# zacz08/ADM

Hardware: AMD Instinct MI355X
Metric: train images/sec (CIFAR-10 32x32 uncond DDM UNet, 1 optimizer step/iter) + 10-step sample images/sec (higher is better)
Workload: dtype f32; 1 GPU; BASELINE configs[1]: CIFAR-10 32x32 uncond two-decoder DhariwalUNet (216M params), bs=128/GPU fp32, ddm_const schedule, dropout 0.1, loss_simple (LPIPS term needs unfetchable VGG16 weights), clip 1.0 + AdamW + EMA(every 8); global_batch=128, image=3x32x32, parallelism=dp1, valid=True

## Files before the change

### adm_amd/csrc/conv_gemm_x6.hip

```cpp
#include "common.h"
#include "../../include/adm_hip.h"

namespace {

struct G6P {
  const float* x; const unsigned short* w; const float* bias; const float* res; float* y;
  int M, N, K, ldx, ldy, ldr, wrows, tilesN, xbytes, wbytes, ybytes, rbytes;
  const float* amax_x; float wscale;
  float* amax_y;
};

typedef __attribute__((address_space(3))) void g6_lds_void;
typedef __bf16 bf16x8 __attribute__((ext_vector_type(8)));
typedef unsigned u32x2 __attribute__((ext_vector_type(2)));
typedef unsigned u32x4 __attribute__((ext_vector_type(4)));
typedef float f32x2 __attribute__((ext_vector_type(2)));
constexpr int GM = 128, GN = 128, GCH = 2;
template <int FMT> struct G6Fmt {
  static constexpr int TERMS = FMT ? 2 : 3;
  static constexpr int IMG = GCH * TERMS * 128 * 16;
  static constexpr int QW = 2 * TERMS;
};
typedef _Float16 g6_f16x8 __attribute__((ext_vector_type(8)));
typedef _Float16 g6_f16x2 __attribute__((ext_vector_type(2)));
__device__ inline float g6_scale(float amax) {
  if (!(amax > 0.f) || !(amax < 3e38f)) return 1.f;
  int e;
  frexpf(16000.f / amax, &e);
  return ldexpf(1.f, e - 1);
}
constexpr int G_RA = 2, G_RB = 4, G_D = 4;

__device__ __forceinline__ f32x4 g6_sub4(f32x4 a, f32x4 b) {
  f32x4 r;
#pragma unroll
  for (int i = 0; i < 4; ++i) asm("v_sub_f32 %0, %1, %2" : "=v"(r[i]) : "v"(a[i]), "v"(b[i]));
  return r;
}
__device__ __forceinline__ void g6_split3(const f32x4 v, u32x2& t0, u32x2& t1, u32x2& t2) {
  f32x4 h, mh;
#pragma unroll
  for (int i = 0; i < 4; ++i) h[i] = __uint_as_float(__float_as_uint(v[i]) & 0xFFFF0000u);
  const f32x4 r = g6_sub4(v, h);
#pragma unroll
  for (int i = 0; i < 4; ++i) mh[i] = __uint_as_float(__float_as_uint(r[i]) & 0xFFFF0000u);
  const f32x4 r2 = g6_sub4(r, mh);
  t0 = u32x2{__builtin_amdgcn_perm(__float_as_uint(v[1]), __float_as_uint(v[0]), 0x07060302u),
             __builtin_amdgcn_perm(__float_as_uint(v[3]), __float_as_uint(v[2]), 0x07060302u)};
  t1 = u32x2{__builtin_amdgcn_perm(__float_as_uint(r[1]), __float_as_uint(r[0]), 0x07060302u),
             __builtin_amdgcn_perm(__float_as_uint(r[3]), __float_as_uint(r[2]), 0x07060302u)};
  t2 = u32x2{__builtin_amdgcn_perm(__float_as_uint(r2[1]), __float_as_uint(r2[0]), 0x07060302u),
             __builtin_amdgcn_perm(__float_as_uint(r2[3]), __float_as_uint(r2[2]), 0x07060302u)};
}
__device__ __forceinline__ void g6_split2(const f32x4 v, float s, u32x2& t0, u32x2& t1) {
  _Float16 h0[4], h1[4];
#pragma unroll
  for (int i = 0; i < 4; ++i) {
    const float vs = v[i] * s;
    h0[i] = (_Float16)vs;
    h1[i] = (_Float16)(vs - (float)h0[i]);
  }
  t0 = u32x2{__builtin_bit_cast(unsigned, g6_f16x2{h0[0], h0[1]}), __builtin_bit_cast(unsigned, g6_f16x2{h0[2], h0[3]})};
  t1 = u32x2{__builtin_bit_cast(unsigned, g6_f16x2{h1[0], h1[1]}), __builtin_bit_cast(unsigned, g6_f16x2{h1[2], h1[3]})};
}
__device__ __forceinline__ void g6_barrier() {
  __builtin_amdgcn_fence(__ATOMIC_RELEASE, "workgroup", "local");
  __builtin_amdgcn_s_barrier();
  __builtin_amdgcn_fence(__ATOMIC_ACQUIRE, "workgroup", "local");
}

template <int FMT>
__global__ __launch_bounds__(512) void gemm_x6_kernel(G6P p) {
  constexpr int G_IMG = G6Fmt<FMT>::IMG, TERMS = G6Fmt<FMT>::TERMS, QW = G6Fmt<FMT>::QW;
  float sa = 1.f, inv_scale = 1.f;
  if (FMT) { sa = g6_scale(adm_amax_read(p.amax_x)); inv_scale = 1.f / (sa * p.wscale); }
  extern __shared__ __attribute__((aligned(16))) unsigned short smg[];
  unsigned short* As = smg;
  unsigned short* Bs = smg + G_RA * G_IMG;
  const int tid = threadIdx.x, lane = tid & 63, hw_wid = tid >> 6;
  const bool producer = hw_wid >= 4;
  const int wid = hw_wid & 3;
  int bid = blockIdx.x;
  {
    const int nwg = gridDim.x, q = nwg >> 3, r = nwg & 7, xcd = bid & 7, idx = bid >> 3;
    bid = (xcd < r ? xcd * (q + 1) : r * (q + 1) + (xcd - r) * q) + idx;
  }
  const int tilesM = gridDim.x / p.tilesN;
  const int tm = bid % tilesM, tn = bid / tilesM;
  const int m0 = tm * GM, n0 = tn * GN;
  const int S = p.K >> 5;
  constexpr unsigned OOB = 0x80000000u;

  if (producer) {
    const __amdgpu_buffer_rsrc_t rs_x = __builtin_amdgcn_make_buffer_rsrc(const_cast<float*>(p.x), 0, p.xbytes, 0x00020000);
    const int ptid = wid * 64 + lane;
    const int prow = ptid >> 3, quad = ptid & 7;
    unsigned voff[4];
#pragma unroll
    for (int j = 0; j < 4; ++j) {
      const int m = m0 + prow + 32 * j;
      voff[j] = (m < p.M) ? (unsigned)(((long)m * p.ldx + quad * 4) * 4) : OOB;
    }
    const int aq = quad & 3, ch = quad >> 2;
    unsigned short* la[4];
#pragma unroll
    for (int j = 0; j < 4; ++j) {
      const int row = prow + 32 * j;
      la[j] = As + (ch * TERMS * 128 + row) * 16 + ((((aq >> 1) ^ (row >> 3)) & 1) << 3) + (aq & 1) * 4;
    }
    f32x4 d[G_D][4];
    auto issue = [&](int set, int s) {
      const int soff = s << 7;
#pragma unroll
      for (int j = 0; j < 4; ++j)
        d[set][j] = __builtin_bit_cast(f32x4, __builtin_amdgcn_raw_buffer_load_b128(rs_x, (int)(s < S ? voff[j] : OOB), soff, 0));
    };
    auto store = [&](int set, int slot) {
#pragma unroll
      for (int j = 0; j < 4; ++j) {
        unsigned short* l = la[j] + slot * G_IMG;
        if (FMT) {
          u32x2 h0, h1;
          g6_split2(d[set][j], sa, h0, h1);
          *reinterpret_cast<u32x2*>(l) = h0;
          *reinterpret_cast<u32x2*>(l + 128 * 16) = h1;
          continue;
        }
        u32x2 t0, t1, t2;
        g6_split3(d[set][j], t0, t1, t2);
        *reinterpret_cast<u32x2*>(l) = t0;
        *reinterpret_cast<u32x2*>(l + 128 * 16) = t1;
        *reinterpret_cast<u32x2*>(l + 2 * 128 * 16) = t2;
      }
    };
#pragma unroll
    for (int k = 0; k < G_D; ++k) issue(k, k);
    __builtin_amdgcn_sched_barrier(0);
    for (int s0 = 0; s0 < S; s0 += G_D) {
#pragma unroll
      for (int k = 0; k < G_D; ++k) {
        if (s0 + k < S) {
          store(k, k & 1);
          __builtin_amdgcn_sched_barrier(0);
          issue(k, s0 + k + G_D);
          __builtin_amdgcn_sched_barrier(0);
          g6_barrier();
        }
      }
    }
    return;
  }

  const __amdgpu_buffer_rsrc_t rs_w = __builtin_amdgcn_make_buffer_rsrc(const_cast<unsigned short*>(p.w), 0, p.wbytes, 0x00020000);
  const int wm = wid >> 1, wn = wid & 1;
  const int lr = lane & 31, lh = lane >> 5;
  unsigned b_voff[QW];
#pragma unroll
  for (int i = 0; i < QW; ++i) {
    const int q = wid * QW + i, img = q >> 2;
    const int row = (q & 3) * 32 + (lane >> 1);
    const int n = n0 + row;
    const int half = (lane ^ (row >> 3)) & 1;
    b_voff[i] = (n < p.wrows) ? (unsigned)((((long)img * p.wrows + n) * 16 + half * 8) * 2) : OOB;
  }
  int ld_s = 0, ld_slot = 0;
  auto issue_b = [&]() {
    const int kb = (ld_s * GCH * TERMS * p.wrows) << 5;
    unsigned short* dst = Bs + ld_slot * G_IMG + (wid * QW) * 512;
#pragma unroll
    for (int i = 0; i < QW; ++i)
      __builtin_amdgcn_raw_ptr_buffer_load_lds(rs_w, (g6_lds_void*)(dst + i * 512), 16, (int)b_voff[i], kb, 0, 0);
    ++ld_s;
    if (++ld_slot == G_RB) ld_slot = 0;
  };

  f32x16 acc[2][2], tot[2][2];
#pragma unroll
  for (int a = 0; a < 2; ++a)
#pragma unroll
    for (int b = 0; b < 2; ++b)
#pragma unroll
      for (int r = 0; r < 16; ++r) tot[a][b][r] = 0.f;
  const int fh = ((lh ^ (lr >> 3)) & 1) * 8;
  const int a_foff = (wm * 64 + lr) * 16 + fh;
  const int b_foff = (wn * 64 + lr) * 16 + fh;
  const f32x16 zero = {0.f, 0.f, 0.f, 0.f, 0.f, 0.f, 0.f, 0.f, 0.f, 0.f, 0.f, 0.f, 0.f, 0.f, 0.f, 0.f};

  issue_b();
  if (S > 1) issue_b();
  if (S > 2) issue_b();
  int slot_b = 0;
  for (int s = 0; s < S; ++s) {
    if (s + 2 < S) { if (FMT) asm volatile("s_waitcnt vmcnt(8) lgkmcnt(0)\n\ts_barrier" ::: "memory"); else asm volatile("s_waitcnt vmcnt(12) lgkmcnt(0)\n\ts_barrier" ::: "memory"); }
    else if (s + 1 < S) { if (FMT) asm volatile("s_waitcnt vmcnt(4) lgkmcnt(0)\n\ts_barrier" ::: "memory"); else asm volatile("s_waitcnt vmcnt(6) lgkmcnt(0)\n\ts_barrier" ::: "memory"); }
    else asm volatile("s_waitcnt vmcnt(0) lgkmcnt(0)\n\ts_barrier" ::: "memory");
    if (s + 3 < S) issue_b();
    const unsigned short* Ab = As + (s & 1) * G_IMG + a_foff;
    const unsigned short* Bb = Bs + slot_b * G_IMG + b_foff;
    if (++slot_b == G_RB) slot_b = 0;
    const bool first = (s & 1) == 0;
#pragma unroll
    for (int ch = 0; ch < GCH; ++ch) {
      bf16x8 a[2][TERMS], b[2][TERMS];
#pragma unroll
      for (int k = 0; k < TERMS; ++k)
#pragma unroll
        for (int blk = 0; blk < 2; ++blk) {
          a[blk][k] = __builtin_bit_cast(bf16x8, *reinterpret_cast<const u32x4*>(Ab + ((ch * TERMS + k) * 128 + blk * 32) * 16));
          b[blk][k] = __builtin_bit_cast(bf16x8, *reinterpret_cast<const u32x4*>(Bb + ((ch * TERMS + k) * 128 + blk * 32) * 16));
        }
#pragma unroll
      for (int mi = 0; mi < 2; ++mi)
#pragma unroll
        for (int ni = 0; ni < 2; ++ni) {
          f32x16 c;
          if (FMT) {
            const g6_f16x8 a0 = __builtin_bit_cast(g6_f16x8, a[mi][0]), a1 = __builtin_bit_cast(g6_f16x8, a[mi][1]);
            const g6_f16x8 b0 = __builtin_bit_cast(g6_f16x8, b[ni][0]), b1 = __builtin_bit_cast(g6_f16x8, b[ni][1]);
            c = __builtin_amdgcn_mfma_f32_32x32x16_f16(a0, b1, (first && ch == 0) ? zero : acc[mi][ni], 0, 0, 0);
            c = __builtin_amdgcn_mfma_f32_32x32x16_f16(a1, b0, c, 0, 0, 0);
            acc[mi][ni] = __builtin_amdgcn_mfma_f32_32x32x16_f16(a0, b0, c, 0, 0, 0);
            continue;
          }
          if (first && ch == 0) c = __builtin_amdgcn_mfma_f32_32x32x16_bf16(a[mi][0], b[ni][TERMS - 1], zero, 0, 0, 0);
          else c = __builtin_amdgcn_mfma_f32_32x32x16_bf16(a[mi][0], b[ni][TERMS - 1], acc[mi][ni], 0, 0, 0);
#ifndef G6_HALF
          c = __builtin_amdgcn_mfma_f32_32x32x16_bf16(a[mi][TERMS - 1], b[ni][0], c, 0, 0, 0);
          c = __builtin_amdgcn_mfma_f32_32x32x16_bf16(a[mi][1], b[ni][1], c, 0, 0, 0);
          c = __builtin_amdgcn_mfma_f32_32x32x16_bf16(a[mi][0], b[ni][1], c, 0, 0, 0);
#endif
          c = __builtin_amdgcn_mfma_f32_32x32x16_bf16(a[mi][1], b[ni][0], c, 0, 0, 0);
          acc[mi][ni] = __builtin_amdgcn_mfma_f32_32x32x16_bf16(a[mi][0], b[ni][0], c, 0, 0, 0);
        }
    }
    if (!first || s + 1 == S) {
#pragma unroll
      for (int mi = 0; mi < 2; ++mi)
#pragma unroll
        for (int ni = 0; ni < 2; ++ni) tot[mi][ni] += acc[mi][ni];
    }
  }

  const __amdgpu_buffer_rsrc_t rs_y = __builtin_amdgcn_make_buffer_rsrc(p.y, 0, p.ybytes, 0x00020000);
  const __amdgpu_buffer_rsrc_t rs_r = __builtin_amdgcn_make_buffer_rsrc(const_cast<float*>(p.res), 0, p.res ? p.rbytes : 0, 0x00020000);
  float am = 0.f;
#pragma unroll
  for (int ni = 0; ni < 2; ++ni) {
    const int n = n0 + wn * 64 + ni * 32 + lr;
    const float bv = (p.bias && n < p.N) ? p.bias[n] : 0.f;
#pragma unroll
    for (int mi = 0; mi < 2; ++mi) {
      const int mb = m0 + wm * 64 + mi * 32 + 4 * lh;
      float rv[16];
      unsigned oy[16];
#pragma unroll
      for (int r = 0; r < 16; ++r) {
        const int m = mb + (r & 3) + 8 * (r >> 2);
        const bool ok = m < p.M && n < p.N;
        oy[r] = ok ? ((unsigned)m * (unsigned)p.ldy + (unsigned)n) * 4u : OOB;
        const unsigned orr = ok ? ((unsigned)m * (unsigned)p.ldr + (unsigned)n) * 4u : OOB;
        rv[r] = __builtin_bit_cast(float, __builtin_amdgcn_raw_buffer_load_b32(rs_r, (int)orr, 0, 0));
      }
#pragma unroll
      for (int r = 0; r < 16; ++r) {
        const float v = (FMT ? tot[mi][ni][r] * inv_scale : tot[mi][ni][r]) + bv + rv[r];
        if (oy[r] != OOB) am = fmaxf(am, fabsf(v));
        __builtin_amdgcn_raw_buffer_store_b32(__builtin_bit_cast(unsigned, v), rs_y, (int)oy[r], 0, 0);
      }
    }
  }
  adm_amax_commit(am, p.amax_y);
}

__global__ void split3_rows_kernel(const float* __restrict__ src, unsigned short* __restrict__ dst, int rows, int cols, int ld) {
  const long total = (long)rows * cols;
  for (long i = blockIdx.x * (long)blockDim.x + threadIdx.x; i < total; i += (long)gridDim.x * blockDim.x) {
    const int n = (int)(i / cols), c = (int)(i - (long)n * cols);
    const float a = src[(long)n * ld + c];
    const unsigned u = __float_as_uint(a);
    const float r = a - __uint_as_float(u & 0xFFFF0000u);
    const unsigned m = __float_as_uint(r);
    const float r2 = r - __uint_as_float(m & 0xFFFF0000u);
    unsigned short* d = dst + ((((long)(c >> 4) * 3) * rows + n) << 4) + (c & 15);
    const long term = (long)rows << 4;
    d[0] = (unsigned short)(u >> 16);
    d[term] = (unsigned short)(m >> 16);
    d[2 * term] = (unsigned short)(__float_as_uint(r2) >> 16);
  }
}

__global__ void split2_rows_kernel(const float* __restrict__ src, unsigned short* __restrict__ dst, int rows, int cols, int ld, float scale,
                                   int* __restrict__ overflow) {
  const long total = (long)rows * cols;
  bool bad = false;
  for (long i = blockIdx.x * (long)blockDim.x + threadIdx.x; i < total; i += (long)gridDim.x * blockDim.x) {
    const int n = (int)(i / cols), c = (int)(i - (long)n * cols);
    const float a = src[(long)n * ld + c] * scale;
    bad |= !(fabsf(a) < 65000.f);
    const _Float16 h0 = (_Float16)a, h1 = (_Float16)(a - (float)h0);
    unsigned short* d = dst + ((((long)(c >> 4) * 2) * rows + n) << 4) + (c & 15);
    d[0] = __builtin_bit_cast(unsigned short, h0);
    d[(long)rows << 4] = __builtin_bit_cast(unsigned short, h1);
  }
  if (bad && overflow) *overflow = 1;
}

}

extern "C" int adm_split3_rows(const float* src, void* dst, int rows, int cols, int ld, hipStream_t stream) {
  if (!src || !dst || rows <= 0 || cols <= 0 || (cols & 15) || ld < cols) return ADM_EINVAL;
  const long total = (long)rows * cols;
  const int grid = (int)((total + 255) / 256 > 4096 ? 4096 : (total + 255) / 256);
  hipLaunchKernelGGL(split3_rows_kernel, dim3(grid), dim3(256), 0, stream, src, static_cast<unsigned short*>(dst), rows, cols, ld);
  ADM_CHECK_LAUNCH();
  return ADM_OK;
}

static int gemm_x6_launch(const float* x, const void* w6, const float* bias, const float* res, float* y, long M, int K, int ldx, int N,
                          int wrows, int ldy, int ldr, hipStream_t stream, const float* amax_x, float wscale, float* amax_y) {
  const bool h3 = amax_x != nullptr;
  if (!x || !w6 || !y || M <= 0 || K <= 0 || (K & 31) || (ldx & 3) || N <= 0 || wrows < N) return ADM_EINVAL;
  if (((uintptr_t)x | (uintptr_t)w6) & 15) return ADM_EINVAL;
  if (h3 && !(wscale > 0.f)) return ADM_EINVAL;
  G6P p;
  p.x = x; p.w = static_cast<const unsigned short*>(w6); p.bias = bias; p.res = res; p.y = y;
  p.amax_x = amax_x; p.wscale = wscale; p.amax_y = amax_y;
  const long xb = M * ldx * 4, wb = (h3 ? 2L : 3L) * wrows * K * 2, yb = M * ldy * 4, rb = res ? M * ldr * 4 : 0;
  if (M >= (1L << 30) || xb >= (1L << 31) || wb >= (1L << 31) || yb >= (1L << 31) || rb >= (1L << 31)) return ADM_EINVAL;
  p.M = (int)M; p.N = N; p.K = K; p.ldx = ldx; p.ldy = ldy; p.ldr = ldr; p.wrows = wrows;
  p.xbytes = (int)xb; p.wbytes = (int)wb; p.ybytes = (int)yb; p.rbytes = (int)rb;
  p.tilesN = adm_cdiv(N, GN);
  constexpr int smem0 = (G_RA + G_RB) * G6Fmt<0>::IMG * (int)sizeof(unsigned short), smem1 = (G_RA + G_RB) * G6Fmt<1>::IMG * (int)sizeof(unsigned short);
  static bool attr_set = false;
  if (!attr_set) {
    if (hipFuncSetAttribute(reinterpret_cast<const void*>(&gemm_x6_kernel<0>), hipFuncAttributeMaxDynamicSharedMemorySize, smem0) != hipSuccess ||
        hipFuncSetAttribute(reinterpret_cast<const void*>(&gemm_x6_kernel<1>), hipFuncAttributeMaxDynamicSharedMemorySize, smem1) != hipSuccess)
      return ADM_ELAUNCH;
    attr_set = true;
  }
  const long grid = (long)adm_cdiv(M, GM) * p.tilesN;
  if (h3) hipLaunchKernelGGL(gemm_x6_kernel<1>, dim3((unsigned)grid), dim3(512), smem1, stream, p);
  else hipLaunchKernelGGL(gemm_x6_kernel<0>, dim3((unsigned)grid), dim3(512), smem0, stream, p);
  ADM_CHECK_LAUNCH();
  return ADM_OK;
}

extern "C" int adm_gemm_x6(const float* x, const void* w6, const float* bias, const float* res, float* y, long M, int K, int ldx, int N,
                           int wrows, int ldy, int ldr, hipStream_t stream) {
  return gemm_x6_launch(x, w6, bias, res, y, M, K, ldx, N, wrows, ldy, ldr, stream, nullptr, 0.f, nullptr);
}
extern "C" int adm_gemm_x6_amax(const float* x, const void* w6, const float* bias, const float* res, float* y, long M, int K, int ldx, int N,
                                int wrows, int ldy, int ldr, float* amax_y, hipStream_t stream) {
  return gemm_x6_launch(x, w6, bias, res, y, M, K, ldx, N, wrows, ldy, ldr, stream, nullptr, 0.f, amax_y);
}
extern "C" int adm_gemm_x6_h3(const float* x, const void* wh, const float* bias, const float* res, float* y, long M, int K, int ldx, int N,
                              int wrows, int ldy, int ldr, const float* amax_x, float wscale, float* amax_y, hipStream_t stream) {
  if (!amax_x) return ADM_EINVAL;
  return gemm_x6_launch(x, wh, bias, res, y, M, K, ldx, N, wrows, ldy, ldr, stream, amax_x, wscale, amax_y);
}
extern "C" int adm_split2_rows_f16(const float* src, void* dst, int rows, int cols, int ld, float scale, int* overflow, hipStream_t stream) {
  if (!src || !dst || rows <= 0 || cols <= 0 || (cols & 15) || ld < cols || !(scale > 0.f)) return ADM_EINVAL;
  const long total = (long)rows * cols;
  const int grid = (int)((total + 255) / 256 > 4096 ? 4096 : (total + 255) / 256);
  hipLaunchKernelGGL(split2_rows_kernel, dim3(grid), dim3(256), 0, stream, src, static_cast<unsigned short*>(dst), rows, cols, ld, scale, overflow);
  ADM_CHECK_LAUNCH();
  return ADM_OK;
}
```

### adm_amd/hip.py

```python
from __future__ import annotations

import ctypes
import os
import subprocess
from ctypes import c_double, c_float, c_int, c_long, c_uint64, c_void_p

import torch

_HERE = os.path.dirname(os.path.abspath(__file__))
LIB_PATH = os.path.join(_HERE, "libadm_hip.so")
_lib = None

P, I, L, F, D, U = c_void_p, c_int, c_long, c_float, c_double, c_uint64
_SIGS = {
    "adm_version": [],
    "adm_conv_fwd": [P, P, P, P, P, I, I, I, I, I, I, I, I, I, I, I, I, P],
    "adm_conv_splitk": [I, I, I],
    "adm_conv_fwd_ws": [P, P, P, P, P, P, L, I, I, I, I, I, I, I, I, I, I, I, P],
    "adm_conv_fwd_strided": [P, P, P, P, P, I, I, I, I, I, I, I, I, I, I, I, I, I, I, P],
    "adm_conv_fwd_wino": [P, P, P, P, P, I, I, I, I, I, I, I, I, I, P],
    "adm_conv_fwd_wino_up": [P, P, P, P, P, I, I, I, I, I, I, I, I, I, P],
    "adm_pack_weight_wino": [P, P, P, I, I, I, I, P],
    "adm_pack_weight_wino2d": [P, P, P, I, I, I, I, P],
    "adm_conv_fwd_wino2d": [P, P, P, P, P, P, L, I, I, I, I, I, I, I, I, I, P],
    "adm_wino2d_splitk": [I, I, I, I, I],
    "adm_wino2d_variant": [I],
    "adm_wino2d_h3_wide": [I],
    "adm_wgrad_h3_blocks": [I],
    "adm_conv_fwd_wino2d_x6": [P, P, P, P, P, P, L, I, I, I, I, I, I, I, I, I, P],
    "adm_conv_fwd_wino2d_x6_up": [P, P, P, P, P, P, L, I, I, I, I, I, I, I, I, I, P],
    "adm_wino2d_x6_splitk": [I, I, I, I, I],
    "adm_split3_bf16": [P, P, I, I, P],
    "adm_split2_f16": [P, P, I, I, F, P, P],
    "adm_conv_fwd_wino2d_h3": [P, P, P, P, P, P, L, I, I, I, I, I, I, I, I, I, P, F, I, P],
    "adm_gemm_x6": [P, P, P, P, P, L, I, I, I, I, I, I, P],
    "adm_gemm_x6_amax": [P, P, P, P, P, L, I, I, I, I, I, I, P, P],
    "adm_gemm_x6_h3": [P, P, P, P, P, L, I, I, I, I, I, I, P, F, P, P],
    "adm_split2_rows_f16": [P, P, I, I, I, F, P, P],
    "adm_split3_rows": [P, P, I, I, I, P],
    "adm_conv_wgrad_x6": [P, P, P, P, I, I, I, I, I, I, I, I, P],
    "adm_conv_wgrad_x6_up": [P, P, P, P, I, I, I, I, I, I, I, I, P],
    "adm_conv_wgrad_x6_ws": [P, P, P, P, I, I, I, I, I, I, I, I, I, P],
    "adm_conv_wgrad_x6_plan": [I, I, I, I, I],
    "adm_gemm_wgrad_x6": [P, P, P, P, L, I, I, I, I, I, P],
    "adm_gemm_wgrad_x6_ws": [P, P, P, P, L, I, I, I, I, I, P],
    "adm_gemm_wgrad_x6_plan": [L, I, I],
    "adm_conv_wgrad_x6_h3": [P, P, P, P, I, I, I, I, I, I, I, I, I, I, P, P, P],
    "adm_gemm_wgrad_x6_h3": [P, P, P, P, L, I, I, I, I, I, I, P, P, P],
    "adm_conv_wgrad_x6_bf16a": [P, P, P, P, I, I, I, I, I, I, I, I, I, P],
    "adm_gemm_wgrad_x6_bf16a": [P, P, P, P, L, I, I, I, I, I, P],
    "adm_conv_wgrad": [P, P, P, I, I, I, I, I, I, I, I, I, I, P],
    "adm_conv_wgrad_wino": [P, P, P, P, I, I, I, I, I, I, I, I, P],
    "adm_conv_wgrad_wino_up": [P, P, P, P, I, I, I, I, I, I, I, I, P],
    "adm_conv_wgrad_bias": [P, P, P, P, I, I, I, I, I, I, I, I, I, I, P],
    "adm_conv_wgrad_wino2d": [P, P, P, P, I, I, I, I, I, I, I, I, P],
    "adm_unpack_wgrad_wino2d": [P, I, P, I, I, I, I, I, P, P, P],
    "adm_conv_wgrad_plan": [I, I, I, I, I, I, I, I],
    "adm_conv_wgrad_ws": [P, P, P, P, I, I, I, I, I, I, I, I, I, I, I, P],
    "adm_unpack_wgrad_splits": [P, I, P, I, I, I, I, I, I, I, P, P, P],
    "adm_conv_fwd_bf16": [P, P, P, P, P, I, I, I, I, I, I, I, I, I, I, I, I, P],
    "adm_conv_wgrad_bf16": [P, P, P, I, I, I, I, I, I, I, I, I, I, P],
    "adm_conv_fwd_bf16a": [P, P, P, P, P, I, I, I, I, I, I, I, I, I, I, I, I, P],
    "adm_conv_wgrad_bf16a": [P, P, P, I, I, I, I, I, I, I, I, I, I, P],
    "adm_gn_fwd_bf16out": [P, P, P, P, P, P, L, P, I, I, I, I, F, I, F, U, P],
    "adm_f32_to_bf16": [P, P, L, P],
    "adm_pack_weight": [P, P, P, I, I, I, I, I, I, P],
    "adm_pack_weight_table": [P, I, L, P],
    "adm_unpack_wgrad_table": [P, I, L, P],
    "adm_gn_bwd_param_table": [P, I, L, P],
    "adm_unpack_wgrad": [P, P, I, I, I, I, I, I, I, P],
    "adm_permute_vec": [P, P, I, I, I, I, P],
    "adm_colsum": [P, P, I, I, I, I, P],
    "adm_gn_splits": [I, I],
    "adm_gn_fused": [I],
    "adm_gn_stats": [P, P, P, I, I, I, I, F, P],
    "adm_gn_apply": [P, P, P, P, P, L, P, I, I, I, I, I, F, U, P],
    "adm_gn_fwd": [P, P, P, P, P, P, L, P, I, I, I, I, F, I, F, U, P],
    "adm_gn_fwd_amax": [P, P, P, P, P, P, L, P, P, I, I, I, I, F, I, F, U, P],
    "adm_gn_bwd": [P, P, P, P, P, P, L, P, P, P, P, P, I, I, I, I, I, F, U, P],
    "adm_gn_bwd_add": [P, P, P, P, P, P, L, P, P, P, P, P, P, I, I, I, I, I, F, U, P],
    "adm_gn_bwd_add_amax": [P, P, P, P, P, P, L, P, P, P, P, P, P, P, I, I, I, I, I, F, U, P],
    "adm_softmax_rows": [P, L, I, L, F, P],
    "adm_posterior_sample": [P, I, P, P, I, L, I, F, P],
    "adm_attn_fwd": [P, P, P, I, I, I, P],
    "adm_attn_bwd": [P, P, P, P, P, P, I, I, I, P],
    "adm_attn_bwd_amax": [P, P, P, P, P, P, P, I, I, I, P],
    "adm_attn_fwd_h3": [P, P, P, P, I, I, I, P],
    "adm_attn_bwd_h3": [P, P, P, P, P, P, P, P, P, I, I, I, P],
    "adm_resample2x": [P, P, I, I, I, I, I, F, I, P],
    "adm_nchw_to_nhwc": [P, I, P, L, P, I, I, I, I, P],
    "adm_nchw_to_nhwc_amax": [P, I, P, L, P, P, I, I, I, I, P],
# ... 70 lines not shown
    "adm_transpose2d": [P, P, I, I, P],
    "adm_adaptive_weight": [P, L, P, L, P, F, P, P],
    "adm_axpy_dev": [P, P, P, F, P, L, P],
    "adm_swin_attn_fwd": [P, P, P, P, I, I, I, I, I, I, I, I, P],
    "adm_ln_affine_fwd": [P, P, P, P, L, I, F, P],
    "adm_swin_merge_ln_fwd": [P, P, P, P, I, I, I, I, F, P],
    "adm_swin_attn_bwd_ws_floats": [I, I, I, I],
    "adm_swin_attn_bwd": [P, P, P, P, P, P, P, P, I, I, I, I, I, I, I, I, I, I, P],
    "adm_ln_bwd_ws_floats": [L, I],
    "adm_ln_affine_bwd": [P, P, P, P, P, P, P, L, I, F, I, P],
    "adm_swin_merge_ln_bwd": [P, P, P, P, P, P, P, I, I, I, I, F, I, P],
    "adm_rowscale_add": [P, P, P, P, I, L, P],
}
EXPORTS = tuple(_SIGS)


def build(verbose: bool = False) -> str:
    r = subprocess.run(["make", "-C", os.path.join(_HERE, "csrc"), "-j8"], capture_output=True, text=True)
    if verbose or r.returncode != 0:
        print(r.stdout[-4000:], r.stderr[-8000:])
    if r.returncode != 0 or not os.path.exists(LIB_PATH):
        raise RuntimeError("building libadm_hip.so failed")
    return LIB_PATH


def lib() -> ctypes.CDLL:
    global _lib
    if _lib is None:
        if not os.path.exists(LIB_PATH):
            raise RuntimeError(f"{LIB_PATH} is missing: run `python -c 'import __graft_entry__ as g; g.build()'` "
                               "(there is no non-HIP fallback for the adm_amd hot path)")
        _lib = ctypes.CDLL(LIB_PATH)
        for name, args in _SIGS.items():
            fn = getattr(_lib, name)
            fn.argtypes = args
            fn.restype = c_long if name in ("adm_aug_workspace_floats", "adm_linattn_ws_floats", "adm_swin_attn_bwd_ws_floats",
                                        "adm_ln_bwd_ws_floats") else c_int
        if os.environ.get("ADM_H3_WIDE") is not None:
            _lib.adm_wino2d_h3_wide(int(os.environ["ADM_H3_WIDE"]))
        if os.environ.get("ADM_WGRAD_H3_BLOCKS") is not None:
            _lib.adm_wgrad_h3_blocks(int(os.environ["ADM_WGRAD_H3_BLOCKS"]))
    return _lib


def stream() -> c_void_p:
    return c_void_p(torch.cuda.current_stream().cuda_stream)


def ptr(t) -> c_void_p:
    return None if t is None else c_void_p(t.data_ptr())


NO_STREAM = ("adm_version", "adm_conv_splitk", "adm_gn_splits", "adm_aug_workspace_floats", "adm_conv_wgrad_plan",
             "adm_sumsq_blocks", "adm_lnc_blocks", "adm_bn_blocks", "adm_linattn_ws_floats", "adm_wino2d_splitk", "adm_wino2d_x6_splitk", "adm_wino2d_variant", "adm_wino2d_h3_wide", "adm_wgrad_h3_blocks", "adm_gn_fused", "adm_conv_wgrad_x6_plan", "adm_gemm_wgrad_x6_plan", "adm_lpips_head_blocks", "adm_ae_blocks", "adm_swin_attn_bwd_ws_floats", "adm_ln_bwd_ws_floats")


def call(name: str, *args):
    rc = getattr(lib(), name)(*args, stream())
    if rc != 0:
        raise RuntimeError(f"{name} failed with code {rc} (-22 = unsupported shape/alignment, -5 = launch failure)")


def require_cuda(t: torch.Tensor, what: str = "tensor"):
    if not t.is_cuda:
        raise RuntimeError(f"adm_amd: {what} is on {t.device}; the HIP hot path needs a GPU tensor "
                           "(no CPU fallback exists by design)")
```

### include/adm_hip.h

```cpp
#ifndef ADM_HIP_H
#define ADM_HIP_H
#include <stdint.h>
typedef struct ihipStream_t* hipStream_t;

#ifdef __cplusplus
#define ADM_AMAX_SLOTS 64
#define ADM_AMAX_STRIDE 32
#define ADM_AMAX_FLOATS (ADM_AMAX_SLOTS * ADM_AMAX_STRIDE)

extern "C" {
#endif

int adm_version(void);


int adm_conv_fwd(const float* x, const float* wp, const float* bias, const float* res, float* y,
                 int B, int H, int W, int Cin, int ldx, int N, int wrows, int ldy, int ldr,
                 int ks, int up, int tile, hipStream_t stream);

int adm_conv_fwd_strided(const float* x, const float* wp, const float* bias, const float* res, float* y,
                         int B, int Hin, int Win, int Hout, int Wout, int Cin, int ldx, int N, int wrows,
                         int ldy, int ldr, int ks, int stride, int pad_lo, hipStream_t stream);

int adm_conv_fwd_wino(const float* x, const float* wq, const float* bias, const float* res, float* y, int B, int H, int W,
                      int Cin, int ldx, int N, int wrows, int ldy, int ldr, hipStream_t stream);
int adm_conv_fwd_wino_up(const float* x, const float* wq, const float* bias, const float* res, float* y, int B, int H, int W,
                         int Cin, int ldx, int N, int wrows, int ldy, int ldr, hipStream_t stream);
int adm_pack_weight_wino(const float* w, float* wf, float* wb, int Co, int Ci, int Co_pad, int Ci_pad, hipStream_t stream);

int adm_conv_splitk(int M, int N, int K);
int adm_conv_fwd_ws(const float* x, const float* wp, const float* bias, const float* res, float* y, float* ws,
                    long ws_floats, int B, int H, int W, int Cin, int ldx, int N, int wrows, int ldy, int ldr, int ks,
                    int up, hipStream_t stream);

int adm_conv_wgrad(const float* x, const float* dy, float* dwp, int B, int H, int W, int Cin, int ldx,
                   int Cout, int lddy, int ks, int up, int splits, hipStream_t stream);

int adm_conv_wgrad_bias(const float* x, const float* dy, float* dwp, float* dbias, int B, int H, int W, int Cin, int ldx,
                        int Cout, int lddy, int ks, int up, int splits, hipStream_t stream);

int adm_conv_wgrad_wino(const float* x, const float* dy, float* dwp, float* dbias, int B, int H, int W, int Cin, int ldx,
                        int Cout, int lddy, int splits, hipStream_t stream);

int adm_conv_wgrad_wino_up(const float* x, const float* dy, float* dwp, float* dbias, int B, int H, int W, int Cin, int ldx,
                           int Cout, int lddy, int splits, hipStream_t stream);

int adm_pack_weight_wino2d(const float* w, float* wf, float* wb, int Co, int Ci, int Co_pad, int Ci_pad, hipStream_t stream);
int adm_conv_fwd_wino2d(const float* x, const float* wq, const float* bias, const float* res, float* y, float* ws, long ws_floats,
                        int B, int H, int W, int Cin, int ldx, int N, int wrows, int ldy, int ldr, hipStream_t stream);
int adm_conv_fwd_wino2d_x6(const float* x, const void* wq6, const float* bias, const float* res, float* y, float* ws,
                           long ws_floats, int B, int H, int W, int Cin, int ldx, int N, int wrows, int ldy, int ldr,
                           hipStream_t stream);
int adm_conv_fwd_wino2d_x6_up(const float* x, const void* wq6, const float* bias, const float* res, float* y, float* ws,
                              long ws_floats, int B, int H, int W, int Cin, int ldx, int N, int wrows, int ldy, int ldr,
                              hipStream_t stream);
int adm_wino2d_x6_splitk(int B, int H, int W, int Cin, int N);
int adm_split2_f16(const float* src, void* dst, int rows, int cols, float scale, int* overflow, hipStream_t stream);
int adm_conv_fwd_wino2d_h3(const float* x, const void* wqh, const float* bias, const float* res, float* y, float* ws,
                           long ws_floats, int B, int H, int W, int Cin, int ldx, int N, int wrows, int ldy, int ldr,
                           const float* amax_x, float wscale, int up, hipStream_t stream);
int adm_split3_bf16(const float* src, void* dst, int rows, int cols, hipStream_t stream);
int adm_gemm_x6(const float* x, const void* w6, const float* bias, const float* res, float* y, long M, int K, int ldx, int N, int wrows,
                int ldy, int ldr, hipStream_t stream);
int adm_split3_rows(const float* src, void* dst, int rows, int cols, int ld, hipStream_t stream);
int adm_gemm_x6_amax(const float* x, const void* w6, const float* bias, const float* res, float* y, long M, int K, int ldx, int N,
                     int wrows, int ldy, int ldr, float* amax_y, hipStream_t stream);
int adm_gemm_x6_h3(const float* x, const void* wh, const float* bias, const float* res, float* y, long M, int K, int ldx, int N, int wrows,
                   int ldy, int ldr, const float* amax_x, float wscale, float* amax_y, hipStream_t stream);
int adm_split2_rows_f16(const float* src, void* dst, int rows, int cols, int ld, float scale, int* overflow, hipStream_t stream);
int adm_conv_wgrad_x6(const float* x, const float* dy, float* dwp2, float* dbias, int B, int H, int W, int Cin, int ldx, int Cout,
                      int lddy, int splits, hipStream_t stream);
int adm_conv_wgrad_x6_up(const float* x, const float* dy, float* dwp2, float* dbias, int B, int H, int W, int Cin, int ldx, int Cout,
                         int lddy, int splits, hipStream_t stream);
int adm_conv_wgrad_x6_ws(const float* x, const float* dy, float* ws, float* bws, int B, int H, int W, int Cin, int ldx, int Cout,
                         int lddy, int splits, int up, hipStream_t stream);
int adm_conv_wgrad_x6_plan(int B, int H, int W, int Cin, int Cout);
int adm_gemm_wgrad_x6(const float* x, const float* dy, float* dwp, float* dbias, long P, int Cin, int ldx, int Cout, int lddy,
                      int splits, hipStream_t stream);
int adm_gemm_wgrad_x6_ws(const float* x, const float* dy, float* ws, float* bws, long P, int Cin, int ldx, int Cout, int lddy,
                         int splits, hipStream_t stream);
int adm_gemm_wgrad_x6_plan(long P, int Cin, int Cout);
int adm_conv_wgrad_x6_bf16a(const void* x16, const float* dy, float* dwp2, float* dbias, int B, int H, int W, int Cin, int ldx,
                            int Cout, int lddy, int splits, int up, hipStream_t stream);
int adm_gemm_wgrad_x6_bf16a(const void* x16, const float* dy, float* dwp, float* dbias, long P, int Cin, int ldx, int Cout, int lddy,
                            int splits, hipStream_t stream);
int adm_conv_wgrad_x6_h3(const float* x, const float* dy, float* dwp2, float* dbias, int B, int H, int W, int Cin, int ldx, int Cout,
                         int lddy, int splits, int up, int det, const float* amax_x, const float* amax_dy, hipStream_t stream);
int adm_gemm_wgrad_x6_h3(const float* x, const float* dy, float* dwp, float* dbias, long P, int Cin, int ldx, int Cout, int lddy,
                         int splits, int det, const float* amax_x, const float* amax_dy, hipStream_t stream);
int adm_wino2d_variant(int ws);
int adm_wino2d_h3_wide(int v);
int adm_wgrad_h3_blocks(int v);
int adm_wino2d_splitk(int B, int H, int W, int Cin, int N);

int adm_conv_wgrad_wino2d(const float* x, const float* dy, float* dwp2, float* dbias, int B, int H, int W, int Cin, int ldx,
                          int Cout, int lddy, int splits, hipStream_t stream);
int adm_unpack_wgrad_wino2d(const float* wx, int splits, float* dw, int Co, int Ci, int Co_pad, int Ci_pad, int accumulate,
                            const float* bws, float* dbias, hipStream_t stream);

int adm_conv_wgrad_plan(int B, int H, int W, int Cin, int Cout, int ks, int up, int wino);
int adm_conv_wgrad_ws(const float* x, const float* dy, float* ws, float* bws, int B, int H, int W, int Cin, int ldx, int Cout,
                      int lddy, int ks, int up, int splits, int wino, hipStream_t stream);

int adm_conv_fwd_bf16(const float* x, const unsigned short* wp16, const float* bias, const float* res, float* y,
                      int B, int H, int W, int Cin, int ldx, int N, int wrows, int ldy, int ldr, int ks, int up,
                      int tile, hipStream_t stream);
int adm_conv_wgrad_bf16(const float* x, const float* dy, float* dwp, int B, int H, int W, int Cin, int ldx, int Cout,
                        int lddy, int ks, int up, int splits, hipStream_t stream);
int adm_conv_fwd_bf16a(const void* x16, const unsigned short* wp16, const float* bias, const float* res, float* y, int B, int H, int W,
                       int Cin, int ldx, int N, int wrows, int ldy, int ldr, int ks, int up, int tile, hipStream_t stream);
int adm_conv_wgrad_bf16a(const void* x16, const float* dy, float* dwp, int B, int H, int W, int Cin, int ldx, int Cout, int lddy, int ks,
                         int up, int splits, hipStream_t stream);
int adm_gn_fwd_bf16out(const float* x, float* stats, double* ws, const float* gamma, const float* beta, const float* ss,
                       long ss_bstride, void* y16, int B, int HW, int C, int G, float eps, int silu, float drop_p, uint64_t seed,
                       hipStream_t stream);
int adm_f32_to_bf16(const float* src, unsigned short* dst, long n, hipStream_t stream);

int adm_pack_weight(const float* w, float* wp_fwd, float* wp_bwd, int Co, int Ci, int ks, int Co_pad, int Ci_pad,
                    int qkv, hipStream_t stream);
int adm_pack_weight_table(const long* table, int n_entries, long total_tiles, hipStream_t stream);
int adm_unpack_wgrad(const float* dwp, float* dw, int Co, int Ci, int ks, int Co_pad, int Ci_pad, int qkv,
                     int accumulate, hipStream_t stream);
// ... 232 lines not shown
```

Baseline: 1249 images/s.

## Make x6 GEMM kernel process multiple output tiles per workgroup to fix wave quantization

The split-bf16 GEMM kernel now lets each workgroup loop over a chunk of T consecutive output tiles instead of exactly one. A host-side planner picks T so the number of rounds over 256 concurrent workgroups is no worse than launching one tile per workgroup. The producer and consumer pipelines carry their K-step and tile counters across tile boundaries, with a full drain barrier at each new tile and the epilogue run per tile. This targets tail-wave imbalance on large tile counts, at the cost of extra index bookkeeping, a pipeline stall at each tile switch, and some ablation macros left in the code.

```diff
diff --git a/adm_amd/csrc/conv_gemm_x6.hip b/adm_amd/csrc/conv_gemm_x6.hip
--- a/adm_amd/csrc/conv_gemm_x6.hip
+++ b/adm_amd/csrc/conv_gemm_x6.hip
@@ -5,7 +5,7 @@
 
 struct G6P {
   const float* x; const unsigned short* w; const float* bias; const float* res; float* y;
-  int M, N, K, ldx, ldy, ldr, wrows, tilesN, xbytes, wbytes, ybytes, rbytes;
+  int M, N, K, ldx, ldy, ldr, wrows, tilesM, tilesN, tiles, T, xbytes, wbytes, ybytes, rbytes;
   const float* amax_x; float wscale;
   float* amax_y;
 };
@@ -30,6 +30,9 @@
   return ldexpf(1.f, e - 1);
 }
 constexpr int G_RA = 2, G_RB = 4, G_D = 4;
+#ifndef G6_ABL
+#define G6_ABL 0
+#endif
 
 __device__ __forceinline__ f32x4 g6_sub4(f32x4 a, f32x4 b) {
   f32x4 r;
@@ -80,27 +83,32 @@
   const int tid = threadIdx.x, lane = tid & 63, hw_wid = tid >> 6;
   const bool producer = hw_wid >= 4;
   const int wid = hw_wid & 3;
-  int bid = blockIdx.x;
+  int c = blockIdx.x;
   {
-    const int nwg = gridDim.x, q = nwg >> 3, r = nwg & 7, xcd = bid & 7, idx = bid >> 3;
-    bid = (xcd < r ? xcd * (q + 1) : r * (q + 1) + (xcd - r) * q) + idx;
-  }
-  const int tilesM = gridDim.x / p.tilesN;
-  const int tm = bid % tilesM, tn = bid / tilesM;
-  const int m0 = tm * GM, n0 = tn * GN;
-  const int S = p.K >> 5;
+    const int nwg = gridDim.x, q = nwg >> 3, r = nwg & 7, xcd = c & 7, idx = c >> 3;
+    c = (xcd < r ? xcd * (q + 1) : r * (q + 1) + (xcd - r) * q) + idx;
+  }
+  const int t0 = c * p.T;
+  const int nT = min(p.T, p.tiles - t0);
+  const int S = (G6_ABL & 1) ? 0 : p.K >> 5;
+  const int G = nT * S;
   constexpr unsigned OOB = 0x80000000u;
 
   if (producer) {
+    if (G6_ABL & 1) return;
     const __amdgpu_buffer_rsrc_t rs_x = __builtin_amdgcn_make_buffer_rsrc(const_cast<float*>(p.x), 0, p.xbytes, 0x00020000);
     const int ptid = wid * 64 + lane;
     const int prow = ptid >> 3, quad = ptid & 7;
+    int is_ = 0, ij = 0, im = t0 % p.tilesM;
     unsigned voff[4];
-#pragma unroll
-    for (int j = 0; j < 4; ++j) {
-      const int m = m0 + prow + 32 * j;
-      voff[j] = (m < p.M) ? (unsigned)(((long)m * p.ldx + quad * 4) * 4) : OOB;
-    }
+    auto tile_rows = [&]() {
+#pragma unroll
+      for (int j = 0; j < 4; ++j) {
+        const int m = im * GM + prow + 32 * j;
+        voff[j] = (ij < nT && m < p.M) ? ((unsigned)m * (unsigned)p.ldx + quad * 4) * 4u : OOB;
+      }
+    };
+    tile_rows();
     const int aq = quad & 3, ch = quad >> 2;
     unsigned short* la[4];
 #pragma unroll
@@ -109,11 +117,16 @@
       la[j] = As + (ch * TERMS * 128 + row) * 16 + ((((aq >> 1) ^ (row >> 3)) & 1) << 3) + (aq & 1) * 4;
     }
     f32x4 d[G_D][4];
-    auto issue = [&](int set, int s) {
-      const int soff = s << 7;
+    auto issue = [&](int set) {
+      const int soff = is_ << 7;
 #pragma unroll
       for (int j = 0; j < 4; ++j)
-        d[set][j] = __builtin_bit_cast(f32x4, __builtin_amdgcn_raw_buffer_load_b128(rs_x, (int)(s < S ? voff[j] : OOB), soff, 0));
+        d[set][j] = __builtin_bit_cast(f32x4, __builtin_amdgcn_raw_buffer_load_b128(rs_x, (int)voff[j], soff, 0));
+      if (++is_ == S) {
+        is_ = 0; ++ij;
+        if (++im == p.tilesM) im = 0;
+        tile_rows();
+      }
     };
     auto store = [&](int set, int slot) {
 #pragma unroll
@@ -126,23 +139,23 @@
           *reinterpret_cast<u32x2*>(l + 128 * 16) = h1;
           continue;
         }
-        u32x2 t0, t1, t2;
-        g6_split3(d[set][j], t0, t1, t2);
-        *reinterpret_cast<u32x2*>(l) = t0;
+        u32x2 t0_, t1, t2;
+        g6_split3(d[set][j], t0_, t1, t2);
+        *reinterpret_cast<u32x2*>(l) = t0_;
         *reinterpret_cast<u32x2*>(l + 128 * 16) = t1;
         *reinterpret_cast<u32x2*>(l + 2 * 128 * 16) = t2;
       }
     };
 #pragma unroll
-    for (int k = 0; k < G_D; ++k) issue(k, k);
+    for (int k = 0; k < G_D; ++k) issue(k);
     __builtin_amdgcn_sched_barrier(0);
-    for (int s0 = 0; s0 < S; s0 += G_D) {
+    for (int g0 = 0; g0 < G; g0 += G_D) {
 #pragma unroll
       for (int k = 0; k < G_D; ++k) {
-        if (s0 + k < S) {
+        if (g0 + k < G) {
           store(k, k & 1);
           __builtin_amdgcn_sched_barrier(0);
-          issue(k, s0 + k + G_D);
+          issue(k);
           __builtin_amdgcn_sched_barrier(0);
           g6_barrier();
         }
@@ -154,24 +167,31 @@
   const __amdgpu_buffer_rsrc_t rs_w = __builtin_amdgcn_make_buffer_rsrc(const_cast<unsigned short*>(p.w), 0, p.wbytes, 0x00020000);
   const int wm = wid >> 1, wn = wid & 1;
   const int lr = lane & 31, lh = lane >> 5;
+  int tm = t0 % p.tilesM, tn = t0 / p.tilesM;
+  int ld_s = 0, ld_slot = 0, ld_tm = tm, ld_tn = tn;
   unsigned b_voff[QW];
-#pragma unroll
-  for (int i = 0; i < QW; ++i) {
-    const int q = wid * QW + i, img = q >> 2;
-    const int row = (q & 3) * 32 + (lane >> 1);
-    const int n = n0 + row;
-    const int half = (lane ^ (row >> 3)) & 1;
-    b_voff[i] = (n < p.wrows) ? (unsigned)((((long)img * p.wrows + n) * 16 + half * 8) * 2) : OOB;
-  }
-  int ld_s = 0, ld_slot = 0;
+  auto tile_cols = [&]() {
+#pragma unroll
+    for (int i = 0; i < QW; ++i) {
+      const int q = wid * QW + i, img = q >> 2;
+      const int row = (q & 3) * 32 + (lane >> 1);
+      const int n = ld_tn * GN + row;
+      const int half = (lane ^ (row >> 3)) & 1;
+      b_voff[i] = (n < p.wrows) ? (unsigned)((((long)img * p.wrows + n) * 16 + half * 8) * 2) : OOB;
+    }
+  };
+  tile_cols();
   auto issue_b = [&]() {
     const int kb = (ld_s * GCH * TERMS * p.wrows) << 5;
     unsigned short* dst = Bs + ld_slot * G_IMG + (wid * QW) * 512;
 #pragma unroll
     for (int i = 0; i < QW; ++i)
       __builtin_amdgcn_raw_ptr_buffer_load_lds(rs_w, (g6_lds_void*)(dst + i * 512), 16, (int)b_voff[i], kb, 0, 0);
-    ++ld_s;
     if (++ld_slot == G_RB) ld_slot = 0;
+    if (++ld_s == S) {
+      ld_s = 0;
+      if (++ld_tm == p.tilesM) { ld_tm = 0; ++ld_tn; tile_cols(); }
+    }
   };
 
   f32x16 acc[2][2], tot[2][2];
@@ -185,89 +205,106 @@
   const int a_foff = (wm * 64 + lr) * 16 + fh;
   const int b_foff = (wn * 64 + lr) * 16 + fh;
   const f32x16 zero = {0.f, 0.f, 0.f, 0.f, 0.f, 0.f, 0.f, 0.f, 0.f, 0.f, 0.f, 0.f, 0.f, 0.f, 0.f, 0.f};
-
-  issue_b();
-  if (S > 1) issue_b();
-  if (S > 2) issue_b();
-  int slot_b = 0;
-  for (int s = 0; s < S; ++s) {
-    if (s + 2 < S) { if (FMT) asm volatile("s_waitcnt vmcnt(8) lgkmcnt(0)\n\ts_barrier" ::: "memory"); else asm volatile("s_waitcnt vmcnt(12) lgkmcnt(0)\n\ts_barrier" ::: "memory"); }
-    else if (s + 1 < S) { if (FMT) asm volatile("s_waitcnt vmcnt(4) lgkmcnt(0)\n\ts_barrier" ::: "memory"); else asm volatile("s_waitcnt vmcnt(6) lgkmcnt(0)\n\ts_barrier" ::: "memory"); }
-    else asm volatile("s_waitcnt vmcnt(0) lgkmcnt(0)\n\ts_barrier" ::: "memory");
-    if (s + 3 < S) issue_b();
-    const unsigned short* Ab = As + (s & 1) * G_IMG + a_foff;
-    const unsigned short* Bb = Bs + slot_b * G_IMG + b_foff;
-    if (++slot_b == G_RB) slot_b = 0;
-    const bool first = (s & 1) == 0;
-#pragma unroll
-    for (int ch = 0; ch < GCH; ++ch) {
-      bf16x8 a[2][TERMS], b[2][TERMS];
-#pragma unroll
-      for (int k = 0; k < TERMS; ++k)
-#pragma unroll
-        for (int blk = 0; blk < 2; ++blk) {
-          a[blk][k] = __builtin_bit_cast(bf16x8, *reinterpret_cast<const u32x4*>(Ab + ((ch * TERMS + k) * 128 + blk * 32) * 16));
-          b[blk][k] = __builtin_bit_cast(bf16x8, *reinterpret_cast<const u32x4*>(Bb + ((ch * TERMS + k) * 128 + blk * 32) * 16));
-        }
-#pragma unroll
-      for (int mi = 0; mi < 2; ++mi)
-#pragma unroll
-        for (int ni = 0; ni < 2; ++ni) {
-          f32x16 c;
-          if (FMT) {
-            const g6_f16x8 a0 = __builtin_bit_cast(g6_f16x8, a[mi][0]), a1 = __builtin_bit_cast(g6_f16x8, a[mi][1]);
-            const g6_f16x8 b0 = __builtin_bit_cast(g6_f16x8, b[ni][0]), b1 = __builtin_bit_cast(g6_f16x8, b[ni][1]);
-            c = __builtin_amdgcn_mfma_f32_32x32x16_f16(a0, b1, (first && ch == 0) ? zero : acc[mi][ni], 0, 0, 0);
-            c = __builtin_amdgcn_mfma_f32_32x32x16_f16(a1, b0, c, 0, 0, 0);
-            acc[mi][ni] = __builtin_amdgcn_mfma_f32_32x32x16_f16(a0, b0, c, 0, 0, 0);
-            continue;
-          }
-          if (first && ch == 0) c = __builtin_amdgcn_mfma_f32_32x32x16_bf16(a[mi][0], b[ni][TERMS - 1], zero, 0, 0, 0);
-          else c = __builtin_amdgcn_mfma_f32_32x32x16_bf16(a[mi][0], b[ni][TERMS - 1], acc[mi][ni], 0, 0, 0);
-#ifndef G6_HALF
-          c = __builtin_amdgcn_mfma_f32_32x32x16_bf16(a[mi][TERMS - 1], b[ni][0], c, 0, 0, 0);
-          c = __builtin_amdgcn_mfma_f32_32x32x16_bf16(a[mi][1], b[ni][1], c, 0, 0, 0);
-          c = __builtin_amdgcn_mfma_f32_32x32x16_bf16(a[mi][0], b[ni][1], c, 0, 0, 0);
-#endif
-          c = __builtin_amdgcn_mfma_f32_32x32x16_bf16(a[mi][1], b[ni][0], c, 0, 0, 0);
-          acc[mi][ni] = __builtin_amdgcn_mfma_f32_32x32x16_bf16(a[mi][0], b[ni][0], c, 0, 0, 0);
-        }
-    }
-    if (!first || s + 1 == S) {
-#pragma unroll
-      for (int mi = 0; mi < 2; ++mi)
-#pragma unroll
-        for (int ni = 0; ni < 2; ++ni) tot[mi][ni] += acc[mi][ni];
-    }
-  }
-
   const __amdgpu_buffer_rsrc_t rs_y = __builtin_amdgcn_make_buffer_rsrc(p.y, 0, p.ybytes, 0x00020000);
   const __amdgpu_buffer_rsrc_t rs_r = __builtin_amdgcn_make_buffer_rsrc(const_cast<float*>(p.res), 0, p.res ? p.rbytes : 0, 0x00020000);
   float am = 0.f;
-#pragma unroll
-  for (int ni = 0; ni < 2; ++ni) {
-    const int n = n0 + wn * 64 + ni * 32 + lr;
-    const float bv = (p.bias && n < p.N) ? p.bias[n] : 0.f;
-#pragma unroll
-    for (int mi = 0; mi < 2; ++mi) {
-      const int mb = m0 + wm * 64 + mi * 32 + 4 * lh;
-      float rv[16];
-      unsigned oy[16];
-#pragma unroll
-      for (int r = 0; r < 16; ++r) {
-        const int m = mb + (r & 3) + 8 * (r >> 2);
-        const bool ok = m < p.M && n < p.N;
-        oy[r] = ok ? ((unsigned)m * (unsigned)p.ldy + (unsigned)n) * 4u : OOB;
-        const unsigned orr = ok ? ((unsigned)m * (unsigned)p.ldr + (unsigned)n) * 4u : OOB;
-        rv[r] = __builtin_bit_cast(float, __builtin_amdgcn_raw_buffer_load_b32(rs_r, (int)orr, 0, 0));
-      }
-#pragma unroll
-      for (int r = 0; r < 16; ++r) {
-        const float v = (FMT ? tot[mi][ni][r] * inv_scale : tot[mi][ni][r]) + bv + rv[r];
-        if (oy[r] != OOB) am = fmaxf(am, fabsf(v));
-        __builtin_amdgcn_raw_buffer_store_b32(__builtin_bit_cast(unsigned, v), rs_y, (int)oy[r], 0, 0);
-      }
-    }
+
+  if (G > 0) issue_b();
+  if (G > 1) issue_b();
+  if (G > 2) issue_b();
+  int g = 0, slot_b = 0;
+  for (int j = 0; j < nT; ++j) {
+    for (int s = 0; s < S; ++s, ++g) {
+      if (s == 0 && j > 0) asm volatile("s_waitcnt vmcnt(0) lgkmcnt(0)\n\ts_barrier" ::: "memory");
+      else if (g + 2 < G) { if (FMT) asm volatile("s_waitcnt vmcnt(8) lgkmcnt(0)\n\ts_barrier" ::: "memory"); else asm volatile("s_waitcnt vmcnt(12) lgkmcnt(0)\n\ts_barrier" ::: "memory"); }
+      else if (g + 1 < G) { if (FMT) asm volatile("s_waitcnt vmcnt(4) lgkmcnt(0)\n\ts_barrier" ::: "memory"); else asm volatile("s_waitcnt vmcnt(6) lgkmcnt(0)\n\ts_barrier" ::: "memory"); }
+      else asm volatile("s_waitcnt vmcnt(0) lgkmcnt(0)\n\ts_barrier" ::: "memory");
+      if (g + 3 < G) issue_b();
+      const unsigned short* Ab = As + (g & 1) * G_IMG + a_foff;
+      const unsigned short* Bb = Bs + slot_b * G_IMG + b_foff;
+      if (++slot_b == G_RB) slot_b = 0;
+      const bool first = (s & 1) == 0;
+#pragma unroll
+      for (int ch = 0; ch < GCH; ++ch) {
+        bf16x8 a[2][TERMS], b[2][TERMS];
+#pragma unroll
+        for (int k = 0; k < TERMS; ++k)
+#pragma unroll
+          for (int blk = 0; blk < 2; ++blk) {
+            a[blk][k] = __builtin_bit_cast(bf16x8, *reinterpret_cast<const u32x4*>(Ab + ((ch * TERMS + k) * 128 + blk * 32) * 16));
+            b[blk][k] = __builtin_bit_cast(bf16x8, *reinterpret_cast<const u32x4*>(Bb + ((ch * TERMS + k) * 128 + blk * 32) * 16));
+          }
+#pragma unroll
+        for (int mi = 0; mi < 2; ++mi)
+#pragma unroll
+          for (int ni = 0; ni < 2; ++ni) {
+            f32x16 c_;
+            if (FMT) {
+              const g6_f16x8 a0 = __builtin_bit_cast(g6_f16x8, a[mi][0]), a1 = __builtin_bit_cast(g6_f16x8, a[mi][1]);
+              const g6_f16x8 b0 = __builtin_bit_cast(g6_f16x8, b[ni][0]), b1 = __builtin_bit_cast(g6_f16x8, b[ni][1]);
+              c_ = __builtin_amdgcn_mfma_f32_32x32x16_f16(a0, b1, (first && ch == 0) ? zero : acc[mi][ni], 0, 0, 0);
+              c_ = __builtin_amdgcn_mfma_f32_32x32x16_f16(a1, b0, c_, 0, 0, 0);
+              acc[mi][ni] = __builtin_amdgcn_mfma_f32_32x32x16_f16(a0, b0, c_, 0, 0, 0);
+              continue;
+            }
+            if (first && ch == 0) c_ = __builtin_amdgcn_mfma_f32_32x32x16_bf16(a[mi][0], b[ni][TERMS - 1], zero, 0, 0, 0);
+            else c_ = __builtin_amdgcn_mfma_f32_32x32x16_bf16(a[mi][0], b[ni][TERMS - 1], acc[mi][ni], 0, 0, 0);
+#ifndef G6_HALF
+            c_ = __builtin_amdgcn_mfma_f32_32x32x16_bf16(a[mi][TERMS - 1], b[ni][0], c_, 0, 0, 0);
+            c_ = __builtin_amdgcn_mfma_f32_32x32x16_bf16(a[mi][1], b[ni][1], c_, 0, 0, 0);
+            c_ = __builtin_amdgcn_mfma_f32_32x32x16_bf16(a[mi][0], b[ni][1], c_, 0, 0, 0);
+#endif
+            c_ = __builtin_amdgcn_mfma_f32_32x32x16_bf16(a[mi][1], b[ni][0], c_, 0, 0, 0);
+            acc[mi][ni] = __builtin_amdgcn_mfma_f32_32x32x16_bf16(a[mi][0], b[ni][0], c_, 0, 0, 0);
+          }
+      }
+      if (!first || s + 1 == S) {
+#pragma unroll
+        for (int mi = 0; mi < 2; ++mi)
+#pragma unroll
+          for (int ni = 0; ni < 2; ++ni) tot[mi][ni] += acc[mi][ni];
+      }
+    }
+
+    const int m0 = tm * GM, n0 = tn * GN;
+    if (++tm == p.tilesM) { tm = 0; ++tn; }
+    if (G6_ABL & 2) {
+      am += tot[0][0][0] + tot[0][1][1] + tot[1][0][2] + tot[1][1][3];
+    } else {
+#pragma unroll
+      for (int ni = 0; ni < 2; ++ni) {
+        const int n = n0 + wn * 64 + ni * 32 + lr;
+        const float bv = (p.bias && n < p.N) ? p.bias[n] : 0.f;
+#pragma unroll
+        for (int mi = 0; mi < 2; ++mi) {
+          const int mb = m0 + wm * 64 + mi * 32 + 4 * lh;
+          float rv[16];
+          unsigned oy[16];
+#pragma unroll
+          for (int r = 0; r < 16; ++r) {
+            const int m = mb + (r & 3) + 8 * (r >> 2);
+            const bool ok = m < p.M && n < p.N;
+            oy[r] = ok ? ((unsigned)m * (unsigned)p.ldy + (unsigned)n) * 4u : OOB;
+            const unsigned orr = ok ? ((unsigned)m * (unsigned)p.ldr + (unsigned)n) * 4u : OOB;
+            rv[r] = __builtin_bit_cast(float, __builtin_amdgcn_raw_buffer_load_b32(rs_r, (int)orr, 0, 0));
+          }
+#pragma unroll
+          for (int r = 0; r < 16; ++r) {
+            const float v = (FMT ? tot[mi][ni][r] * inv_scale : tot[mi][ni][r]) + bv + rv[r];
+            if (oy[r] != OOB) am = fmaxf(am, fabsf(v));
+            __builtin_amdgcn_raw_buffer_store_b32(__builtin_bit_cast(unsigned, v), rs_y, (int)oy[r], 0, 0);
+          }
+        }
+      }
+    }
+#pragma unroll
+    for (int a = 0; a < 2; ++a)
+#pragma unroll
+      for (int b = 0; b < 2; ++b) tot[a][b] = zero;
+  }
+  if (G6_ABL & 2) {
+    if (p.M < 0) p.y[tid] = am;
+    return;
   }
   adm_amax_commit(am, p.amax_y);
 }
@@ -316,6 +353,23 @@
   return ADM_OK;
 }
 
+static int g_gemm_chunk = 0;
+static int gemm_x6_chunk_plan(long tiles) {
+  if (tiles <= 256) return 1;
+  int best = 1;
+  long cost = (tiles + 255) / 256;
+  for (int T = 2; T <= 8; ++T) {
+    const long wgs = (tiles + T - 1) / T, ct = (wgs + 255) / 256 * T;
+    if (ct <= cost) { cost = ct; best = T; }
+  }
+  return best;
+}
+extern "C" int adm_gemm_x6_plan(long M, int N) {
+  if (M <= 0 || N <= 0) return ADM_EINVAL;
+  return gemm_x6_chunk_plan((long)adm_cdiv(M, GM) * adm_cdiv(N, GN));
+}
+extern "C" int adm_gemm_x6_chunk(int t) { const int old = g_gemm_chunk; if (t >= 0 && t <= 8) g_gemm_chunk = t; return old; }
+
 static int gemm_x6_launch(const float* x, const void* w6, const float* bias, const float* res, float* y, long M, int K, int ldx, int N,
                           int wrows, int ldy, int ldr, hipStream_t stream, const float* amax_x, float wscale, float* amax_y) {
   const bool h3 = amax_x != nullptr;
@@ -329,7 +383,11 @@
   if (M >= (1L << 30) || xb >= (1L << 31) || wb >= (1L << 31) || yb >= (1L << 31) || rb >= (1L << 31)) return ADM_EINVAL;
   p.M = (int)M; p.N = N; p.K = K; p.ldx = ldx; p.ldy = ldy; p.ldr = ldr; p.wrows = wrows;
   p.xbytes = (int)xb; p.wbytes = (int)wb; p.ybytes = (int)yb; p.rbytes = (int)rb;
-  p.tilesN = adm_cdiv(N, GN);
+  p.tilesM = adm_cdiv(M, GM); p.tilesN = adm_cdiv(N, GN);
+  const long tiles = (long)p.tilesM * p.tilesN;
+  if (tiles >= (1L << 31)) return ADM_EINVAL;
+  p.tiles = (int)tiles;
+  p.T = g_gemm_chunk ? g_gemm_chunk : gemm_x6_chunk_plan(tiles);
   constexpr int smem0 = (G_RA + G_RB) * G6Fmt<0>::IMG * (int)sizeof(unsigned short), smem1 = (G_RA + G_RB) * G6Fmt<1>::IMG * (int)sizeof(unsigned short);
   static bool attr_set = false;
   if (!attr_set) {
@@ -338,7 +396,7 @@
       return ADM_ELAUNCH;
     attr_set = true;
   }
-  const long grid = (long)adm_cdiv(M, GM) * p.tilesN;
+  const long grid = (tiles + p.T - 1) / p.T;
   if (h3) hipLaunchKernelGGL(gemm_x6_kernel<1>, dim3((unsigned)grid), dim3(512), smem1, stream, p);
   else hipLaunchKernelGGL(gemm_x6_kernel<0>, dim3((unsigned)grid), dim3(512), smem0, stream, p);
   ADM_CHECK_LAUNCH();
diff --git a/adm_amd/hip.py b/adm_amd/hip.py
--- a/adm_amd/hip.py
+++ b/adm_amd/hip.py
@@ -37,6 +37,8 @@
     "adm_gemm_x6_amax": [P, P, P, P, P, L, I, I, I, I, I, I, P, P],
     "adm_gemm_x6_h3": [P, P, P, P, P, L, I, I, I, I, I, I, P, F, P, P],
     "adm_split2_rows_f16": [P, P, I, I, I, F, P, P],
+    "adm_gemm_x6_plan": [L, I],
+    "adm_gemm_x6_chunk": [I],
     "adm_split3_rows": [P, P, I, I, I, P],
     "adm_conv_wgrad_x6": [P, P, P, P, I, I, I, I, I, I, I, I, P],
     "adm_conv_wgrad_x6_up": [P, P, P, P, I, I, I, I, I, I, I, I, P],
@@ -213,7 +215,7 @@
 
 
 NO_STREAM = ("adm_version", "adm_conv_splitk", "adm_gn_splits", "adm_aug_workspace_floats", "adm_conv_wgrad_plan",
-             "adm_sumsq_blocks", "adm_lnc_blocks", "adm_bn_blocks", "adm_linattn_ws_floats", "adm_wino2d_splitk", "adm_wino2d_x6_splitk", "adm_wino2d_variant", "adm_wino2d_h3_wide", "adm_wgrad_h3_blocks", "adm_gn_fused", "adm_conv_wgrad_x6_plan", "adm_gemm_wgrad_x6_plan", "adm_lpips_head_blocks", "adm_ae_blocks", "adm_swin_attn_bwd_ws_floats", "adm_ln_bwd_ws_floats")
+             "adm_sumsq_blocks", "adm_lnc_blocks", "adm_bn_blocks", "adm_linattn_ws_floats", "adm_wino2d_splitk", "adm_wino2d_x6_splitk", "adm_wino2d_variant", "adm_wino2d_h3_wide", "adm_wgrad_h3_blocks", "adm_gn_fused", "adm_conv_wgrad_x6_plan", "adm_gemm_wgrad_x6_plan", "adm_gemm_x6_plan", "adm_gemm_x6_chunk", "adm_lpips_head_blocks", "adm_ae_blocks", "adm_swin_attn_bwd_ws_floats", "adm_ln_bwd_ws_floats")
 
 
 def call(name: str, *args):
diff --git a/include/adm_hip.h b/include/adm_hip.h
--- a/include/adm_hip.h
+++ b/include/adm_hip.h
@@ -68,6 +68,8 @@
 int adm_gemm_x6_h3(const float* x, const void* wh, const float* bias, const float* res, float* y, long M, int K, int ldx, int N, int wrows,
                    int ldy, int ldr, const float* amax_x, float wscale, float* amax_y, hipStream_t stream);
 int adm_split2_rows_f16(const float* src, void* dst, int rows, int cols, int ld, float scale, int* overflow, hipStream_t stream);
+int adm_gemm_x6_plan(long M, int N);
+int adm_gemm_x6_chunk(int t);
 int adm_conv_wgrad_x6(const float* x, const float* dy, float* dwp2, float* dbias, int B, int H, int W, int Cin, int ldx, int Cout,
                       int lddy, int splits, hipStream_t stream);
 int adm_conv_wgrad_x6_up(const float* x, const float* dy, float* dwp2, float* dbias, int B, int H, int W, int Cin, int ldx, int Cout,
```

After: 1251 images/s, median of 3. Within noise of the previous version (+0.1%).
